# mohsij/spacecraft-pose-estimation

Hardware: AMD Instinct MI355X
Metric: poses/sec end-to-end (HRNet+PnP) at batch 256; keypoint/pose err vs ref (higher is better)
Workload: dtype bf16

## Files before the change

### spacecraft-pose-estimation_amd/csrc/api.cpp

```cpp
#include "common.h"
#include <new>

using namespace scpose;

struct scpose_conv { PackedConv pc; };

extern "C" int32_t scpose_abi_version(void) { return SCPOSE_ABI_VERSION; }
extern "C" int32_t scpose_is_dev_build(void) { return scpose::kDevBuild ? 1 : 0; }
extern "C" const char* scpose_last_error(void) { return last_error(); }

extern "C" int32_t scpose_decode(const float* heatmaps, int32_t n, int32_t j, int32_t h, int32_t w,
                                 const float* center, const float* scale, int32_t post_process,
                                 float* preds_xyc, void* stream) {
  if (n == 0) return SCPOSE_OK;
  SCP_REQUIRE(heatmaps && preds_xyc, "decode: null argument");
  return decode_launch(heatmaps, n, j, h, w, center, scale, post_process, preds_xyc, nullptr,
                       nullptr, static_cast<hipStream_t>(stream));
}

extern "C" int32_t scpose_crop_warp(const uint8_t* frames, const int64_t* offsets, const int32_t* frame_hw,
                                    const double* minv, int32_t n, int32_t out_h, int32_t out_w, int32_t swap_rb,
                                    uint8_t* crops, void* stream) {
  if (n == 0) return SCPOSE_OK;
  SCP_REQUIRE(frames && offsets && frame_hw && minv && crops, "crop_warp: null argument");
// ... 398 lines not shown
}

extern "C" int32_t scpose_conv_create(const float* weight, const float* bias, int32_t cout,
                                      int32_t cin, int32_t ksize, int32_t stride, int32_t dtype,
                                      scpose_conv_t* out) {
  SCP_REQUIRE(weight && out, "conv_create: null argument");
  scpose_conv* c = new (std::nothrow) scpose_conv();
  if (!c) { set_error("conv_create: out of host memory"); return SCPOSE_E_NOMEM; }
  const int32_t rc = conv_upload(weight, bias, cout, cin, ksize, stride, dtype, &c->pc);
  if (rc != SCPOSE_OK) { conv_free(&c->pc); delete c; return rc; }
  *out = c;
  return SCPOSE_OK;
}

extern "C" int32_t scpose_conv_destroy(scpose_conv_t c) {
  if (!c) return SCPOSE_OK;
  conv_free(&c->pc);
  delete c;
  return SCPOSE_OK;
}

extern "C" int32_t scpose_conv_forward(scpose_conv_t c, const void* in, int32_t n, int32_t h,
                                       int32_t w, const void* residual, int32_t relu,
                                       int32_t out_nchw_f32, void* out, void* stream) {
  SCP_REQUIRE(c && in && out, "conv_forward: null argument");
  return conv_launch(c->pc, in, n, h, w, residual, relu, out_nchw_f32, out,
                     static_cast<hipStream_t>(stream));
}

extern "C" int32_t scpose_basic_block_forward(scpose_conv_t conv1, scpose_conv_t conv2, const void* in, int32_t n,
                                              int32_t h, int32_t w, void* out, void* stream) {
  SCP_REQUIRE(conv1 && conv2 && in && out, "basic_block_forward: null argument");
  SCP_REQUIRE(block_fusable(conv1->pc, conv2->pc), "basic_block_forward: not a fusable pair (3x3 stride-1 C->C->C, C = 32 or 48)");
  return block_launch(conv1->pc, conv2->pc, in, n, h, w, out, static_cast<hipStream_t>(stream));
}

extern "C" int32_t scpose_fuse_sum(const void* const* terms, const int32_t* shifts, int32_t nterms,
                                   int32_t n, int32_t c, int32_t h, int32_t w, int32_t dtype,
                                   void* out, void* stream) {
  SCP_REQUIRE(terms && shifts && out, "fuse_sum: null argument");
  return fuse_sum_launch(terms, shifts, nterms, n, c, h, w, dtype, out,
                         static_cast<hipStream_t>(stream));
}

extern "C" int32_t scpose_nchw_f32_to_blocked(const float* src, int32_t n, int32_t c, int32_t h,
                                              int32_t w, int32_t dtype, void* dst, void* stream) {
  SCP_REQUIRE(src && dst, "nchw_f32_to_blocked: null argument");
  return nchw_to_blocked_launch(src, n, c, h, w, dtype, dst, static_cast<hipStream_t>(stream));
}

extern "C" int32_t scpose_blocked_to_nchw_f32(const void* src, int32_t n, int32_t c, int32_t h,
                                              int32_t w, int32_t dtype, float* dst, void* stream) {
  SCP_REQUIRE(src && dst, "blocked_to_nchw_f32: null argument");
  return blocked_to_nchw_launch(src, n, c, h, w, dtype, dst, static_cast<hipStream_t>(stream));
}
```

### spacecraft-pose-estimation_amd/csrc/common.h

```cpp
#pragma once
#include <hip/hip_runtime.h>
#include <stdint.h>
#include <stddef.h>
#include <string>
#include <vector>
#include <string.h>

#include "../../include/scpose.h"

namespace scpose {

void set_error(const char* fmt, ...);
const char* dev_env(const char* name);
const char* last_error();

#define SCP_CHECK_HIP(expr)                                                         \
  do {                                                                              \
    hipError_t _e = (expr);                                                         \
    if (_e != hipSuccess) {                                                         \
      ::scpose::set_error("%s failed: %s (%s:%d)", #expr, hipGetErrorString(_e),    \
                          __FILE__, __LINE__);                                      \
      return SCPOSE_E_HIP;                                                          \
    }                                                                               \
  } while (0)
// ... 109 lines not shown
  float* d_b1 = nullptr;
  size_t w1_bytes = 0;
  int cout_pad1 = 0;
  struct TileMemo { int n = -1, ho = 0, wo = 0, cus = 0; M32Tiling t; };
  mutable TileMemo m32_memo[2];
  void* d_ws2 = nullptr;
  float* d_bs2 = nullptr;
};
bool conv_s2r_config(int cin, int cout, int stride, int* planes, int* nblk, int* g);
size_t conv_s2r_pack(const float* w, int cout, int cin, int dtype, uint16_t* dst);
void conv_s2r_pack_bias(const float* bias, int cout, float* dst);
int32_t conv_s2r_launch(const PackedConv& pc, const void* in, int N, int H, int W, int relu, void* out, hipStream_t stream);
bool conv1x1_stream_eligible(const PackedConv& pc);
int32_t conv1x1_stream_launch(const PackedConv& pc, const void* in, int N, int H, int W, const void* res, int relu,
                              void* out, hipStream_t stream);

void choose_mrep_cp(int cin, int cout, int ks, int stride, int* mrep, int* cp);
void choose_tile(int ks, int stride, int Ho, int Wo, int* nrep, int* th, int* tw);

size_t pack_conv_weights(const float* w, int cout, int cin, int ks, int mt, int cp, int dtype,
                         uint16_t* dst, int* nchunks, int* ksteps_full);

int32_t conv_upload(const float* w, const float* bias, int cout, int cin, int ks, int stride,
                    int dtype, PackedConv* pc);
void conv_free(PackedConv* pc);
int32_t conv_launch(const PackedConv& pc, const void* in, int N, int H, int W, const void* res,
                    int relu, int out_nchw_f32, void* out, hipStream_t stream, int cu_share = 0);
size_t conv_lds_bytes(const PackedConv& pc, int nrep, int th, int tw);
int plane_stride_for(int stride, int halo_h, int halo_w);
int32_t conv_launch_pipe(const PackedConv& pc, ConvLaunch& L, int nrep, int nt, int occ, int groups, hipStream_t stream);
size_t conv_pipe_lds_bytes(const PackedConv& pc, int plane_stride, int groups);
const void* conv_zero_page();
bool block_fusable(const PackedConv& c1, const PackedConv& c2);
int32_t block_launch(const PackedConv& c1, const PackedConv& c2, const void* in, int N, int H, int W, void* out,
                     hipStream_t stream);
int conv_device_cus();
unsigned long long* conv_dbg_buffer(hipStream_t stream);
void conv_dbg_set_grid(int grid);
constexpr int kMrep48 = 15;
bool conv_m32_choose(int cin, int cout, int ks, int stride, int* mr, int* wm, int* cp);
size_t pack_conv_weights_m32(const float* w, int cout, int cin, int ks, int mt, int cp, int dtype,
                             uint16_t* dst, int* nchunks, int* ksteps_full);
int32_t conv_launch_m32(const PackedConv& pc, ConvLaunch& L, hipStream_t stream);

void stem_fused_pack(const float* w1, const float* b1, const float* w2, const float* b2, int dtype, std::vector<uint16_t>* pw1,
                     std::vector<uint16_t>* pw2, std::vector<float>* pb1, std::vector<float>* pb2);
int32_t stem_fused_launch(const void* in, int in_fmt, const void* w1, const void* w2, const float* b1, const float* b2,
                          const float* mean_std, int N, int H, int W, int dtype, void* out,
                          uint32_t* sched , hipStream_t stream);

bool bottleneck_fusable(int cin, int cmid, int cout);
void bottleneck_pack(const float* w1, const float* w2, const float* w3, const float* wds, const float* b1, const float* b2, const float* b3,
                     const float* bds, int cin, int dtype,
                     std::vector<uint16_t>* pw1, std::vector<uint16_t>* pw2, std::vector<uint16_t>* pw3, std::vector<float>* pb);
int32_t bottleneck_launch(const void* in, const void* w1, const void* w2, const void* w3, const float* bias, int N, int H, int W,
                          int cin, int dtype, void* out, uint32_t* sched ,
                          hipStream_t stream);

struct FuseDownPacked {
  void* d_w = nullptr;
  float* d_b = nullptr;
  int c0 = 0, nb = 0, dtype = 0;
};
bool fuse_down_supported(int nb, int c0, int c1);
int32_t fuse_down_upload(const float* w, const float* bias, int nb, int c0, int dtype, FuseDownPacked* fd);
void fuse_down_free(FuseDownPacked* fd);
int32_t fuse_down_launch(const FuseDownPacked& fd, const void* x0, int N, int H, int W, const void* const* terms, void* y,
                         void* const* outs, hipStream_t stream);
// ... 73 lines not shown
```

### spacecraft-pose-estimation_amd/csrc/conv_block.hip

```cpp
#include <stdlib.h>
#include <type_traits>

#include "conv_block2_kernel.h"

namespace scpose {

bool block_fusable(const PackedConv& c1, const PackedConv& c2) {
  static const char* e = dev_env("SCPOSE_FUSE_BLOCK");
  if (e && atoi(e) == 0) return false;
  const int C = c1.cin;
  return c1.variant == 0 && c2.variant == 0 && c1.ks == 3 && c2.ks == 3 && c1.stride == 1 && c2.stride == 1 &&
         c1.cout == C && c2.cin == C && c2.cout == C && (C == 48 || C == 32) && c1.mt == C && c2.mt == C &&
         c1.nchunks == 1 && c2.nchunks == 1 && c1.n_mblk == 1 && c2.n_mblk == 1 && c1.dtype == c2.dtype &&
         c1.ksteps_full == block_ksteps(C / 16) && block_lds_bytes(C / 16) <= 160 * 1024;
}

int32_t block_launch(const PackedConv& c1, const PackedConv& c2, const void* in, int N, int H, int W, void* out,
                     hipStream_t stream) {
  SCP_REQUIRE(block_fusable(c1, c2), "block: the two convolutions are not a fusable BasicBlock");
  SCP_REQUIRE(N > 0 && H > 0 && W > 0, "block: bad shape N=%d H=%d W=%d", N, H, W);
  BlockLaunch L;
  L.in = in; L.w1 = c1.d_w; L.w2 = c2.d_w; L.b1 = c1.d_bias; L.b2 = c2.d_bias; L.out = out;
  L.zero16 = conv_zero_page();
  SCP_REQUIRE(L.zero16, "block: cannot allocate the zero page");
  {
    static const char* e = dev_env("SCPOSE_M32_BUF");
    const size_t bytes = (size_t)N * (c1.cin / 8) * H * W * 16;
    L.bytes = (bytes < 0xfffffff0ull && !(e && atoi(e) == 0)) ? (uint32_t)bytes : 0;
  }
  L.N = N; L.H = H; L.W = W;
  L.tiles_x = (W + kBlockTile - 1) / kBlockTile;
  L.tiles_y = (H + kBlockTile - 1) / kBlockTile;
  L.tiles_total = N * L.tiles_x * L.tiles_y;
  L.fd_tiles_img = make_fastdiv(L.tiles_x * L.tiles_y);
  L.fd_tiles_x = make_fastdiv(L.tiles_x);
  int grid = conv_device_cus();
  if (grid > L.tiles_total) grid = L.tiles_total;
  L.tiles_per_wg = (L.tiles_total + grid - 1) / grid;
  L.grid = (L.tiles_total + L.tiles_per_wg - 1) / L.tiles_per_wg;
  { static const char* e = dev_env("SCPOSE_DBG"); const int dbg = (kDevBuild && e) ? atoi(e) : 0;
    L.dbg_buf = (dbg & 8) ? conv_dbg_buffer(stream) : nullptr;
    if (dbg & 8) conv_dbg_set_grid(L.grid); }
  const int mrep = c1.cin / 16;
  static const char* v1 = dev_env("SCPOSE_BLOCK_V1");
  if (L.bytes != 0 && !(v1 && atoi(v1))) {
    if (c1.dtype == SCPOSE_DT_BF16) return mrep == 3 ? block2_launch_one<0, 3>(L, stream) : block2_launch_one<0, 2>(L, stream);
    return mrep == 3 ? block2_launch_one<1, 3>(L, stream) : block2_launch_one<1, 2>(L, stream);
  }
  if (c1.dtype == SCPOSE_DT_BF16) {
    if (mrep == 3) return block_launch_one<0, 3>(L, stream);
    return block_launch_one<0, 2>(L, stream);
  }
  if (mrep == 3) return block_launch_one<1, 3>(L, stream);
  return block_launch_one<1, 2>(L, stream);
}

}
```

### spacecraft-pose-estimation_amd/csrc/conv_block2_kernel.h

```cpp
#pragma once
#include "conv_block_kernel.h"

namespace scpose {

constexpr size_t block2_lds_bytes(int mrep) { return 1024 + 2 * 2 * mrep * (size_t)(block_xs() + block_ms()) + (size_t)mrep * 256 * 16; }

template <int DT, int MREP>
__global__ __launch_bounds__(512, 2) void conv_block2_kernel(const BlockLaunch p) {
  extern __shared__ __attribute__((aligned(16))) char smem[];
  typedef typename DtOf<DT>::type T;
  typedef typename FragOf<T>::type frag_t;
  constexpr int MT = 16 * MREP, PLANES = 2 * MREP, KSTEPS = block_ksteps(MREP), NPT = MREP * 9;
  constexpr int XS = block_xs(), MS = block_ms();
  char* const xl0 = smem + 1024;
  char* const ml0 = xl0 + 2 * PLANES * XS;
  char* const rl0 = ml0 + 2 * PLANES * MS;

  const int tid = threadIdx.x, lane = tid & 63, wave = __builtin_amdgcn_readfirstlane(tid >> 6);
  const int q = lane >> 4, r = lane & 15, half = lane >> 5, psel = q & 1, hi = q >> 1;
  const int role = wave >> 2, rw = wave & 3, rtid = tid & 255;
  const int HW = p.H * p.W;
  const int tiles_per_img = p.tiles_x * p.tiles_y;

  const char* wsrc = static_cast<const char*>(role ? p.w2 : p.w1);
  frag_t wf[KSTEPS][MREP];
#pragma unroll
  for (int s = 0; s < KSTEPS; ++s)
#pragma unroll
    for (int m = 0; m < MREP; ++m)
      wf[s][m] = *reinterpret_cast<const frag_t*>(wsrc + (size_t)s * (4 * MT * 16) + (q * MT + m * 16 + r) * 16);
  float* const bias_l = reinterpret_cast<float*>(smem) + role * 64;
  if (tid < MT) { reinterpret_cast<float*>(smem)[tid] = p.b1[tid]; reinterpret_cast<float*>(smem)[64 + tid] = p.b2[tid]; }

  const int wg = xcd_remap(blockIdx.x, p.grid);
  const int t_begin = wg * p.tiles_per_wg;
  const int t_end = min(p.tiles_total, t_begin + p.tiles_per_wg);
  const int ntiles = t_end - t_begin;
  auto decode = [&](int t, int& img, int& oy0, int& ox0) {
    img = pipe_fdiv(t, p.fd_tiles_img);
    const int rem = t - img * tiles_per_img;
    const int ty = pipe_fdiv(rem, p.fd_tiles_x);
    oy0 = ty * kBlockTile; ox0 = (rem - ty * p.tiles_x) * kBlockTile;
  };
  const buf_rsrc_t rs_in = make_buf(p.in, p.bytes), rs_out = make_buf(p.out, p.bytes);

  auto x_voff = [&](int t, int i) -> uint32_t {
    int img, oy0, ox0;
    decode(t, img, oy0, ox0);
    int rt = rtid;
    asm volatile("" : "+v"(rt));
    const int slot = rt + 256 * i;
    const int hy = slot / 20, hx = slot - hy * 20;
    const int iy = oy0 - 2 + hy, ix = ox0 - 2 + hx;
    const bool ok = iy >= 0 && iy < p.H && ix >= 0 && ix < p.W;
    return ok ? (uint32_t)(img * PLANES * HW + iy * p.W + ix) * 16u : BUF_OOB;
  };
  auto x_dma = [&](uint32_t voff, int i, int pl, int b) {
    if (rtid + 256 * i < 400)
      dma16_buf(rs_in, voff, (uint32_t)(pl * HW) * 16u, xl0 + b * (PLANES * XS) + pl * XS + (rw * 64 + 256 * i) * 16);
  };
  auto issue_x = [&](int t, int b) {
#pragma unroll
    for (int i = 0; i < 2; ++i) {
      const uint32_t voff = x_voff(t, i);
#pragma unroll
      for (int pl = 0; pl < PLANES; ++pl) x_dma(voff, i, pl, b);
    }
  };

  auto koff = [](int pt, int PS, int ROWW) constexpr -> int {
    return pt < NPT ? 2 * (pt / 9) * PS + ((pt % 9) / 3 * ROWW + (pt % 9) % 3) * 16 : 0;
  };

  auto kloop = [&](auto ncol_c, auto role_c, const char* tile, const int* pixoff, f32x4 (*acc)[3], auto&& side, int psel_k) {
    constexpr int NCOL = decltype(ncol_c)::value;
    constexpr int ROLE = decltype(role_c)::value;
    constexpr int PS = ROLE ? MS : XS, ROWW = ROLE ? 18 : 20;
// ... 17 lines not shown
    static_for<0, KSTEPS>([&](auto sc) {
      constexpr int S = decltype(sc)::value;
      fetch(std::integral_constant<int, S + 2>{});
      __builtin_amdgcn_sched_barrier(0);
#pragma unroll
      for (int m = 0; m < MREP; ++m)
#pragma unroll
        for (int n = 0; n < NCOL; ++n) acc[m][n] = mfma16<T>(wf[S][m], bf[S % 3][n], acc[m][n]);
      side(sc);
      __builtin_amdgcn_sched_barrier(0);
    });
  };

  if (role == 1 && ntiles > 0) issue_x(t_begin, 0);
  asm volatile("s_waitcnt vmcnt(0)" ::: "memory");
  __syncthreads();

  unsigned long long tph[6] = {0, 0, 0, 0, 0, 0};
  auto now = [&]() -> unsigned long long {
    if (!SCP_DBG_BUF(p)) return 0ull;
    unsigned long long t;
    asm volatile("s_memtime %0\n\ts_waitcnt lgkmcnt(0)" : "=s"(t) : : "memory");
    return t;
  };
  if (role == 0) {
    for (int i = 0; i <= ntiles; ++i) {
      if (i < ntiles) {
        const int t = t_begin + i;
        int img, oy0, ox0;
        decode(t, img, oy0, ox0);
        const char* xl = xl0 + (i & 1) * (PLANES * XS);
        char* ml = ml0 + (i & 1) * (PLANES * MS);
        const bool narrow = i > 0 && ox0 > 0;
#pragma unroll 1
        for (int pass = 0; pass < 3; ++pass) {
          int rr = r;
          asm volatile("" : "+v"(rr));
          auto geom = [&](int n, int& pidx, int& my, int& mx) {
            const int c = rw + 4 * (2 * pass + n);
            pidx = narrow ? (c < 18 ? c * 18 + 2 + rr : 18 * 18) : c * 16 + rr;
            const bool ok = pidx < 18 * 18;
            my = ok ? pidx / 18 : 0;
            mx = ok ? pidx - my * 18 : 0;
          };
          const int cmax = narrow ? 18 : 21;
          const int ncol = (rw + 8 * pass < cmax) + (rw + 8 * pass + 4 < cmax);
          if (ncol == 0) continue;
          int pixoff[2];
#pragma unroll
          for (int n = 0; n < 2; ++n) {
            int pidx, my, mx;
            geom(n, pidx, my, mx);
            pixoff[n] = (my * 20 + mx) * 16;
          }
          f32x4 acc[MREP][3];
#pragma unroll
          for (int m = 0; m < MREP; ++m) {
            const float4 b4 = *reinterpret_cast<const float4*>(bias_l + m * 16 + q * 4);
#pragma unroll
            for (int n = 0; n < 2; ++n) acc[m][n] = f32x4{b4.x, b4.y, b4.z, b4.w};
          }
          const unsigned long long s1 = now();
          auto none = [](auto) {};
          if (ncol == 2) kloop(std::integral_constant<int, 2>{}, std::integral_constant<int, 0>{}, xl, pixoff, acc, none, psel);
          else kloop(std::integral_constant<int, 1>{}, std::integral_constant<int, 0>{}, xl, pixoff, acc, none, psel);
          const unsigned long long s2 = now();
          tph[1] += s2 - s1;
#pragma unroll
          for (int n = 0; n < 2; ++n) {
            int pidx, my, mx;
            asm volatile("" : "+v"(rr));
            geom(n, pidx, my, mx);
            const int gy = oy0 - 1 + my, gx = ox0 - 1 + mx;
            const bool inimg = gy >= 0 && gy < p.H && gx >= 0 && gx < p.W;
            const bool okn = pidx < 18 * 18 && n < ncol;
#pragma unroll
            for (int m = 0; m < MREP; ++m) {
              uint2 o;
              o.x = relu2_16(pack2<T>(acc[m][n][0], acc[m][n][1]), 0u);
              o.y = relu2_16(pack2<T>(acc[m][n][2], acc[m][n][3]), 0u);
              if (!inimg) o = make_uint2(0u, 0u);
              if (okn) *reinterpret_cast<uint2*>(ml + (2 * m + psel) * MS + pidx * 16 + 8 * hi) = o;
            }
          }
          tph[2] += now() - s2;
        }
      }
      const unsigned long long s9 = now();
      asm volatile("s_waitcnt lgkmcnt(0)\n\ts_barrier" ::: "memory");
      tph[5] += now() - s9;
    }
  } else {
    u32x4 res0[MREP];
#pragma unroll
    for (int m = 0; m < MREP; ++m) res0[m] = u32x4{0u, 0u, 0u, 0u};
    for (int i = 0; i <= ntiles; ++i) {
      const unsigned long long s0 = now();
      if (i == 0 && 1 < ntiles) issue_x(t_begin + 1, 1);
      if (i >= 1 && i < ntiles) {
        int img1, oy1, ox1;
        decode(t_begin + i, img1, oy1, ox1);
        int rt = rtid;
        asm volatile("" : "+v"(rt));
        if (ox1 > 0 && rt < PLANES * 36) {
          const int kpl = rt / 36, krem = rt - kpl * 36;
          const u32x4 keep = *reinterpret_cast<const u32x4*>(ml0 + ((i - 1) & 1) * (PLANES * MS) + kpl * MS + ((krem >> 1) * 18 + 16 + (krem & 1)) * 16);
          *reinterpret_cast<u32x4*>(ml0 + (i & 1) * (PLANES * MS) + kpl * MS + ((krem >> 1) * 18 + (krem & 1)) * 16) = keep;
        }
      }
      tph[0] += now() - s0;
      if (i >= 1) {
        const int t = t_begin + i - 1;
        int img, oy0, ox0;
        decode(t, img, oy0, ox0);
        const char* ml = ml0 + ((i - 1) & 1) * (PLANES * MS);
        auto conv2_pass = [&](auto pass_c) {
          constexpr int pass = decltype(pass_c)::value;
          const int row0 = rw + 8 * pass, row1 = row0 + 4;
          int rt2 = tid;
          asm volatile("" : "+v"(rt2));
          const int rr = rt2 & 15, half_ = (rt2 >> 5) & 1, psel_ = (rt2 >> 4) & 1;
          const int oy = oy0 + (half_ ? row1 : row0), ox = ox0 + rr;
// ... 95 lines not shown
```

### spacecraft-pose-estimation_amd/csrc/conv_block_kernel.h

```cpp
#pragma once
#include "common.h"
#include "conv_device.h"
#include "conv_pipe_kernel.h"

namespace scpose {

struct BlockLaunch {
  const void* in;
  const void* w1;
  const void* w2;
  const float* b1;
  const float* b2;
  void* out;
  const void* zero16;
  uint32_t bytes;
  int32_t N, H, W;
  int32_t tiles_x, tiles_y, tiles_total, tiles_per_wg, grid;
  FastDiv fd_tiles_img, fd_tiles_x;
  unsigned long long* dbg_buf;
};

template <int S, int E, typename F>
__device__ __forceinline__ void static_for(F&& f) {
  if constexpr (S < E) {
    f(std::integral_constant<int, S>{});
    static_for<S + 1, E>(f);
  }
}

constexpr int kBlockTile = 16;
constexpr int block_ksteps(int mrep) { return (mrep * 9 + 1) / 2; }
constexpr int block_xs() { return 20 * 20 * 16; }
constexpr int block_ms() { return (18 * 18 * 16 + 255) & ~255; }
constexpr size_t block_lds_bytes(int mrep) {
  return 1024 + 2 * (size_t)block_ksteps(mrep) * 4 * (16 * mrep) * 16 + 2 * mrep * (size_t)(block_xs() + block_ms());
}

template <int DT, int MREP>
__global__ __launch_bounds__(512, 2) void conv_block_kernel(const BlockLaunch p) {
  extern __shared__ __attribute__((aligned(16))) char smem[];
  typedef typename DtOf<DT>::type T;
  typedef typename FragOf<T>::type frag_t;
  constexpr int MT = 16 * MREP, PLANES = 2 * MREP, KSTEPS = block_ksteps(MREP), NPT = MREP * 9;
  constexpr int XS = block_xs(), MS = block_ms();
  constexpr int WBYTES = KSTEPS * 4 * MT * 16;

  int* koffA = reinterpret_cast<int*>(smem);
  int* koffB = koffA + 64;
  float* bias1 = reinterpret_cast<float*>(smem + 512);
  float* bias2 = bias1 + 64;
  char* w1l = smem + 1024;
  char* w2l = w1l + WBYTES;
// ... 275 lines not shown
```

### spacecraft-pose-estimation_amd/csrc/conv_pipe.hip

```cpp
#include <stdio.h>
#include <stdlib.h>
#include <vector>

#include "common.h"

namespace scpose {

int32_t conv_pipe_dispatch_bf16(int ks, int stride, int mrep, int nrep, int nt, int occ, const ConvLaunch& L, size_t lds, hipStream_t st);
int32_t conv_pipe_dispatch_f16(int ks, int stride, int mrep, int nrep, int nt, int occ, const ConvLaunch& L, size_t lds, hipStream_t st);

int32_t conv_stag_dispatch_bf16(int mrep, int nrep, const ConvLaunch& L, size_t lds, hipStream_t st);
int32_t conv_stag_dispatch_f16(int mrep, int nrep, const ConvLaunch& L, size_t lds, hipStream_t st);

static void* g_zero_page[16] = {nullptr};
static unsigned long long* g_dbg_buf = nullptr;
static int g_dbg_grid = 0;

const void* conv_zero_page() {
  int dev = 0;
  if (hipGetDevice(&dev) != hipSuccess || dev < 0 || dev >= 16) return nullptr;
  if (!g_zero_page[dev]) {
    void* p = nullptr;
    if (hipMalloc(&p, 256) != hipSuccess) return nullptr;
    if (hipMemset(p, 0, 256) != hipSuccess) return nullptr;
// ... 59 lines not shown
  L.items_per_wg = (L.items_total + grid - 1) / grid;
  L.grid = (L.items_total + L.items_per_wg - 1) / L.items_per_wg;
  g_dbg_grid = L.grid;
  if (groups == 2) {
    if (pc.dtype == SCPOSE_DT_BF16) return conv_stag_dispatch_bf16(pc.mrep, nrep, L, lds, stream);
    return conv_stag_dispatch_f16(pc.mrep, nrep, L, lds, stream);
  }
  if (pc.dtype == SCPOSE_DT_BF16) return conv_pipe_dispatch_bf16(pc.ks, pc.stride, pc.mrep, nrep, nt, occ, L, lds, stream);
  return conv_pipe_dispatch_f16(pc.ks, pc.stride, pc.mrep, nrep, nt, occ, L, lds, stream);
}

}

extern "C" void scpose_dbg_dump(void) {
  using namespace scpose;
  if (!g_dbg_buf || g_dbg_grid <= 0) return;
  (void)hipDeviceSynchronize();
  const int n = g_dbg_grid * 8 * 6;
  std::vector<unsigned long long> h(n);
  (void)hipMemcpy(h.data(), g_dbg_buf, n * 8, hipMemcpyDeviceToHost);
  const char* names[6] = {"setup+residual+DMA issue", "MFMA loop", "vmcnt wait", "finalize", "barrier", "stores"};
  double tot = 0, sum[6] = {0};
  int nw = 0;
  for (int i = 0; i < g_dbg_grid * 8; ++i) { double t = 0; for (int k = 0; k < 6; ++k) { sum[k] += (double)h[i * 6 + k]; t += (double)h[i * 6 + k]; } nw += t > 0; }
  for (int k = 0; k < 6; ++k) tot += sum[k];
  printf("  (%d workgroups, %d waves with stamps)\n", g_dbg_grid, nw);
  for (int k = 0; k < 6; ++k) printf("  %-26s %10.0f cycles/wave  %5.1f%%\n", names[k], sum[k] / (nw ? nw : 1), 100 * sum[k] / tot);
  for (int role = 0; role < 2; ++role) {
    double rs[6] = {0}; int rn = 0;
    for (int b = 0; b < g_dbg_grid; ++b)
      for (int w = role * 4; w < role * 4 + 4; ++w) { double t = 0; for (int k = 0; k < 6; ++k) { rs[k] += (double)h[(b * 8 + w) * 6 + k]; t += (double)h[(b * 8 + w) * 6 + k]; } rn += t > 0; }
    if (rn) { printf("  waves %d-%d:", role * 4, role * 4 + 3); for (int k = 0; k < 6; ++k) printf(" %9.0f", rs[k] / rn); printf("\n"); }
  }
}
```

### spacecraft-pose-estimation_amd/csrc/conv_pipe_kernel.h

```cpp
#pragma once
#include "common.h"
#include "conv_device.h"

namespace scpose {

typedef __attribute__((address_space(3))) void lds_void_t;
typedef const __attribute__((address_space(1))) void gbl_void_t;
typedef unsigned int u32x4 __attribute__((ext_vector_type(4)));

__device__ __forceinline__ int pipe_fdiv(int n, const FastDiv& f) {
  return (int)((__umulhi((uint32_t)n, f.mul) + (uint32_t)n * f.add) >> f.shift);
}

__device__ __forceinline__ void dma16(const void* g, void* l_wave_base) {
  __builtin_amdgcn_global_load_lds((gbl_void_t*)g, (lds_void_t*)l_wave_base, 16, 0, 0);
}

constexpr uint32_t BUF_OOB = 0xfffffff0u;
#if defined(__HIP_DEVICE_COMPILE__)
typedef __amdgpu_buffer_rsrc_t buf_rsrc_t;
__device__ __forceinline__ buf_rsrc_t make_buf(const void* base, uint32_t bytes) {
  return __builtin_amdgcn_make_buffer_rsrc(const_cast<void*>(base), 0, bytes, 0x00020000);
}
__device__ __forceinline__ void dma16_buf(buf_rsrc_t r, uint32_t voff, uint32_t soff, void* l_wave_base) {
  __builtin_amdgcn_raw_ptr_buffer_load_lds(r, (lds_void_t*)l_wave_base, 16, voff, soff, 0, 0);
}
__device__ __forceinline__ void store16_buf(buf_rsrc_t r, uint32_t voff, uint32_t soff, u32x4 v) {
  __builtin_amdgcn_raw_buffer_store_b128(v, r, voff, soff, 0);
  asm volatile("s_nop 1" ::"v"(v) : "memory");
}
__device__ __forceinline__ u32x4 load16_buf(buf_rsrc_t r, uint32_t voff, uint32_t soff) {
  return __builtin_amdgcn_raw_buffer_load_b128(r, voff, soff, 0);
}
__device__ __forceinline__ void store4_buf(buf_rsrc_t r, uint32_t voff, uint32_t v) {
  __builtin_amdgcn_raw_buffer_store_b32(v, r, voff, 0u, 0);
}
#else
struct buf_rsrc_t {};
__device__ inline buf_rsrc_t make_buf(const void*, uint32_t) { return buf_rsrc_t{}; }
__device__ inline void dma16_buf(buf_rsrc_t, uint32_t, uint32_t, void*) {}
__device__ inline void store16_buf(buf_rsrc_t, uint32_t, uint32_t, u32x4) {}
__device__ inline u32x4 load16_buf(buf_rsrc_t, uint32_t, uint32_t) { return u32x4{0u, 0u, 0u, 0u}; }
__device__ inline void store4_buf(buf_rsrc_t, uint32_t, uint32_t) {}
#endif

template <int DT, int KS, int STRIDE, int MREP, int NREP, int NT, int OCC, int G>
__global__ __launch_bounds__(256 * G, (G == 2) ? 2 : OCC) void conv_pipe_kernel(const ConvLaunch p) {
  static_assert(G == 1 || NT == 1, "parallel tile groups and sequential tile groups are exclusive");
  extern __shared__ __attribute__((aligned(16))) char smem[];
  typedef typename DtOf<DT>::type T;
  typedef typename FragOf<T>::type frag_t;
  constexpr int MT = 16 * MREP;
  constexpr int MAXP = (STRIDE == 1) ? 2 : 3;
  constexpr int KK = KS * KS;
  constexpr int NPAIR = (NREP + 1) / 2;

  int* koff = reinterpret_cast<int*>(smem);
  float* bias_l = reinterpret_cast<float*>(smem + 512);
  char* wl0 = smem + 512 + p.lds_bias;
  char* xl0 = wl0 + p.nbuf_w * p.lds_w;

  const int lane = threadIdx.x & 63;
  const int wave_all = __builtin_amdgcn_readfirstlane(threadIdx.x >> 6);
  const int grp = wave_all >> 2;
  const int wave = wave_all & 3, tid = threadIdx.x & 255;
  const int q = lane >> 4, r = lane & 15;
  const int HW = p.H * p.W;
  const int HP = p.halo_h * p.halo_w;
  const int npix = p.th * p.tw;
  const int planes_last = p.cin_planes - (p.nchunks - 1) * p.cp;
  const bool w_resident = p.nbuf_w == 1;

  if (threadIdx.x < 128) {
    const int tbl = threadIdx.x >> 6, e = threadIdx.x & 63;
// ... 442 lines not shown
```

### spacecraft-pose-estimation_amd/csrc/hrnet.cpp

```cpp
#include <math.h>
#include <stdio.h>
#include <stdarg.h>
#include <new>

#include <algorithm>
#include <map>
#include <string>
#include <vector>

#include "common.h"

namespace scpose {

static const double kBnEps = 1e-5;

struct HostTensor { const float* p; int64_t n; };

struct Weights {
  std::map<std::string, HostTensor> m;
  bool allow_missing;
  std::string missing;

  const float* get(const std::string& k, int64_t numel) {
    auto it = m.find(k);
// ... 51 lines not shown
  int epoch, lane;
  int par_kind;
};

}

struct scpose_hrnet_lanes {
  hipStream_t side[3] = {nullptr, nullptr, nullptr};
  std::vector<hipEvent_t> fork;
  std::vector<hipEvent_t> join;
  unsigned kinds = 0xe;
};

struct scpose_hrnet {
  scpose_hrnet_desc desc;
  int device = 0;
  std::vector<scpose::PackedConv> convs;
  float* d_mean_std = nullptr;
  void* d_stemf_w1 = nullptr;
  void* d_stemf_w2 = nullptr;
  float* d_stemf_b1 = nullptr;
  float* d_stemf_b2 = nullptr;
  struct Bneck { void* w1 = nullptr; void* w2 = nullptr; void* w3 = nullptr; float* bias = nullptr; int cin = 256; };
  std::vector<Bneck> bnecks;
  std::vector<scpose::FuseDownPacked> fdowns;
  float* d_head_bias = nullptr;
  uint32_t* d_sched = nullptr;
  int head_k = 0, head_s = 1;
  struct HeadFused { bool ok = false; int fuse_op = -1, conv_op = -1; void* d_w = nullptr; float* d_b = nullptr;
                     bool active = false; } headf;
  std::vector<scpose::TensorDesc> tensors;
  std::vector<scpose::Op> ops;
  std::vector<std::pair<std::string, int>> taps;
  struct Plan { int n = -1, h = -1, w = -1; size_t bytes = 0, part_off = 0; std::vector<size_t> off; } plan[2];
  std::vector<hipEvent_t> events;
  bool events_valid = false;
};

namespace scpose {

struct Builder {
  scpose_hrnet* net;
  Weights* W;
  int32_t status = SCPOSE_OK;
  int epoch = 0, lane = 0;
  bool serial = true;
  int par_kind = 0;
  void push(Op op) {
    if (serial) ++epoch;
    op.epoch = epoch; op.lane = serial ? 0 : lane; op.par_kind = serial ? 0 : par_kind;
    net->ops.push_back(op);
  }
  void parallel_begin(int kind) { ++epoch; serial = false; lane = 0; par_kind = kind; }
  void parallel_end() { serial = true; lane = 0; }

  int new_tensor(int C, int ds, const std::string& name) {
    net->tensors.push_back(TensorDesc{C, ds, -1});
    const int t = (int)net->tensors.size() - 1;
    if (!name.empty()) net->taps.emplace_back(name, t);
    return t;
  }
  void rename_tap(int t, const std::string& name) { for (auto& tp : net->taps) if (tp.second == t) tp.first = name; }
  void drop_tap(int t) {
    for (size_t i = 0; i < net->taps.size(); ++i) if (net->taps[i].second == t) { net->taps.erase(net->taps.begin() + i); --i; }
  }
  static std::string tensor_name(const std::string& cname) {
    return cname.size() > 2 && cname.compare(cname.size() - 2, 2, ".0") == 0 ? cname.substr(0, cname.size() - 2) : cname;
// ... 409 lines not shown
        for (size_t j = 0; j < freel.size() && !merged; ++j)
          if (i != j && freel[i].off + freel[i].size == freel[j].off) {
            freel[i].size += freel[j].size;
            freel.erase(freel.begin() + j);
            merged = true;
          }
    }
  };
  P.off.assign(net->tensors.size(), 0);
  std::vector<char> released(net->tensors.size(), 0);
  std::vector<int> pending;
  int cur_epoch = net->ops.empty() ? 0 : net->ops[0].epoch;
  for (size_t i = 0; i < net->ops.size(); ++i) {
    const Op& op = net->ops[i];
    if (mode == 1 && op.epoch != cur_epoch) {
      for (int t : pending) release(P.off[t], tensor_bytes(net->tensors[t], n, h, w));
      pending.clear();
      cur_epoch = op.epoch;
    }
    if (op.out >= 0) P.off[op.out] = alloc(tensor_bytes(net->tensors[op.out], n, h, w));
    for (int k = 0; k < op.nouts; ++k) P.off[op.outs[k]] = alloc(tensor_bytes(net->tensors[op.outs[k]], n, h, w));
    auto done = [&](int t) {
      if (t >= 0 && net->tensors[t].last_use == (int)i && !released[t]) {
        released[t] = 1;
        if (mode == 1) pending.push_back(t);
        else release(P.off[t], tensor_bytes(net->tensors[t], n, h, w));
      }
    };
    done(op.in); done(op.res);
    for (int k = 0; k < op.nterms; ++k) done(op.term[k]);
  }
  P.part_off = top;
  if (net->headf.ok) top += 2 * head_fused_part_bytes(n);
  P.n = n; P.h = h; P.w = w; P.bytes = top;
  return top;
}

struct HeadDecode {
  const float* center;
  const float* scale;
  int post_process;
  float* preds;
};

bool hrnet_tail_fused(const scpose_hrnet* net, int n, int h, int w) {
  if (!net->headf.ok) return false;
  static const char* e = dev_env("SCPOSE_NO_HEAD_FUSE");
  const Op& fo = net->ops[net->headf.fuse_op];
  const TensorDesc& ty = net->tensors[fo.out];
  return !(e && atoi(e)) && head_fused_supported(fo.nterms, ty.C, net->desc.num_joints, n, h >> ty.ds, w >> ty.ds);
}

int32_t hrnet_forward(scpose_hrnet* net, const void* in, int in_fmt, int n, int h, int w,
                      float* heatmaps, void* ws, size_t ws_bytes, hipStream_t st, bool profile, int stop_tensor = -1,
                      int mode = 0, const scpose_hrnet_lanes* lanes = nullptr, const HeadDecode* dec = nullptr) {
  SCP_REQUIRE(n > 0, "hrnet_forward: batch %d", n);
  const bool fused_tail = hrnet_tail_fused(net, n, h, w) && stop_tensor != net->ops[net->headf.fuse_op].out;
  net->headf.active = fused_tail;
  SCP_REQUIRE(heatmaps || (dec && fused_tail) || stop_tensor >= 0,
              "hrnet_forward: this network's tail is not fused for this shape -- key points need a heat-map buffer");
  SCP_REQUIRE(h % 32 == 0 && w % 32 == 0 && h > 0 && w > 0, "hrnet_forward: H=%d W=%d must be multiples of 32", h, w);
  const size_t need = hrnet_plan(net, n, h, w, mode);
  if (ws_bytes < need || !ws) {
    set_error("hrnet_forward: workspace %zu bytes < required %zu", ws_bytes, need);
    return SCPOSE_E_WORKSPACE;
  }
// ... 47 lines not shown
      const void* terms[4];
      for (int k = 0; k < fo.nterms; ++k) terms[k] = ptr(fo.term[k]);
      rc = head_fused_launch(terms, fo.shift, fo.nterms, n, ty.C, h >> ty.ds, w >> ty.ds, net->desc.num_joints, net->desc.dtype,
                             net->headf.d_w, net->headf.d_b, heatmaps, dec ? part_v : nullptr,
                             dec ? part_i : nullptr, dec ? dec->center : nullptr, dec ? dec->scale : nullptr,
                             dec ? dec->post_process : 0, dec ? dec->preds : nullptr, st);
    } else if (op.kind == OP_STEM2) {
      rc = stem_fused_launch(in, in_fmt, net->d_stemf_w1, net->d_stemf_w2, net->d_stemf_b1, net->d_stemf_b2, net->d_mean_std,
                             n, h, w, net->desc.dtype, ptr(op.out), net->d_sched + 16 * oi, st);
    } else if (op.kind == OP_CONV) {
      const TensorDesc& ti = net->tensors[op.in];
      void* out = op.out == -2 ? static_cast<void*>(heatmaps) : ptr(op.out);
      rc = conv_launch(net->convs[op.conv], ptr(op.in), n, h >> ti.ds, w >> ti.ds, ptr(op.res),
                       op.relu, op.out_f32, out, st, open_lanes ? conv_device_cus() / 2 : 0);
    } else if (op.kind == OP_HEAD) {
      const TensorDesc& ti = net->tensors[op.in];
      float* out = op.out == -2 ? heatmaps : static_cast<float*>(ptr(op.out));
      rc = head_gather_launch(ptr(op.in), net->d_head_bias + op.head * 16, static_cast<const float*>(ptr(op.res)), n,
                              net->desc.num_joints, h >> ti.ds, w >> ti.ds, net->head_k, net->head_s,
                              net->desc.dtype, out, st);
    } else if (op.kind == OP_BNECK) {
      const TensorDesc& ti = net->tensors[op.in];
      const scpose_hrnet::Bneck& bn = net->bnecks[op.conv];
      rc = bottleneck_launch(ptr(op.in), bn.w1, bn.w2, bn.w3, bn.bias, n, h >> ti.ds, w >> ti.ds, bn.cin, net->desc.dtype, ptr(op.out), net->d_sched + 16 * oi, st);
    } else if (op.kind == OP_FDOWN) {
      const TensorDesc& ti = net->tensors[op.in];
      const void* terms[3] = {nullptr, nullptr, nullptr};
      void* outs[3] = {nullptr, nullptr, nullptr};
      for (int k = 0; k < op.nterms; ++k) terms[k] = ptr(op.term[k]);
      for (int k = 0; k < op.nouts; ++k) outs[k] = ptr(op.outs[k]);
      rc = fuse_down_launch(net->fdowns[op.conv], ptr(op.in), n, h >> ti.ds, w >> ti.ds, terms, ptr(op.out), outs, st);
    } else if (op.kind == OP_BLOCK) {
      const TensorDesc& ti = net->tensors[op.in];
      rc = block_launch(net->convs[op.conv], net->convs[op.conv2], ptr(op.in), n, h >> ti.ds, w >> ti.ds, ptr(op.out), st);
    } else {
      const TensorDesc& to = net->tensors[op.out];
      const void* terms[4];
      for (int k = 0; k < op.nterms; ++k) terms[k] = ptr(op.term[k]);
      rc = fuse_sum_launch(terms, op.shift, op.nterms, n, to.C, h >> to.ds, w >> to.ds,
                           net->desc.dtype, ptr(op.out), st);
    }
    if (rc != SCPOSE_OK) return rc;
    if (stop_tensor >= 0 && (op.out == stop_tensor || (op.nouts > 0 && std::find(op.outs, op.outs + op.nouts, stop_tensor) != op.outs + op.nouts)))
      break;
  }
  if (lanes) { const int32_t rc = join_lanes(); if (rc != SCPOSE_OK) return rc; }
  st = st0;
  if (dec && !fused_tail && stop_tensor < 0) {
    int32_t hh = 0, hw = 0;
    hh = h / 4 * net->head_s; hw = w / 4 * net->head_s;
    const int32_t rc = decode_launch(heatmaps, n, net->desc.num_joints, hh, hw, dec->center, dec->scale, dec->post_process,
                                     dec->preds, nullptr, nullptr, st);
    if (rc != SCPOSE_OK) return rc;
  }
  if (profile) {
    SCP_CHECK_HIP(hipEventRecord(net->events[opi], st));
    net->events_valid = true;
  }
  return SCPOSE_OK;
}

static void op_work(const scpose_hrnet* net, const Op& op, int h, int w, double* f, double* by, int32_t sig[4], bool unfused = false) {
  *f = 0; *by = 0;
  sig[0] = op.kind; sig[1] = sig[2] = sig[3] = 0;
  if (!unfused && net->headf.active && &op == &net->ops[net->headf.fuse_op]) {
    const TensorDesc& to = net->tensors[op.out];
    sig[1] = op.nterms; sig[2] = to.C; sig[3] = to.C;
// ... 381 lines not shown
```

Measured before the change: 9830.

## Carry halo rows of fused BasicBlock intermediate between vertically adjacent tiles

In the fused two-conv BasicBlock kernel, each workgroup now saves the bottom two rows of its conv1 intermediate tile to a per-workgroup global strip buffer. When it later processes the tile directly below, it DMAs those rows back into LDS instead of recomputing them, so fewer halo columns/passes of conv1 are computed. This adds strip stores, a vmcnt wait at the barrier, scratch buffer planning per lane, and a stream-keyed allocator for the standalone API. It also adds a per-wave debug print.

Result: no change. 9892 (median of 6 runs) (+0.6%).

```diff
diff --git a/spacecraft-pose-estimation_amd/csrc/api.cpp b/spacecraft-pose-estimation_amd/csrc/api.cpp
--- a/spacecraft-pose-estimation_amd/csrc/api.cpp
+++ b/spacecraft-pose-estimation_amd/csrc/api.cpp
@@ -454,7 +454,10 @@
                                               int32_t h, int32_t w, void* out, void* stream) {
   SCP_REQUIRE(conv1 && conv2 && in && out, "basic_block_forward: null argument");
   SCP_REQUIRE(block_fusable(conv1->pc, conv2->pc), "basic_block_forward: not a fusable pair (3x3 stride-1 C->C->C, C = 32 or 48)");
-  return block_launch(conv1->pc, conv2->pc, in, n, h, w, out, static_cast<hipStream_t>(stream));
+  const size_t strip_bytes = block_strip_bytes(conv1->pc.cin, n, h, w);
+  void* strip = strip_bytes ? block_strip_scratch(static_cast<hipStream_t>(stream), strip_bytes) : nullptr;
+  SCP_REQUIRE(!strip_bytes || strip, "basic_block_forward: cannot allocate %zu bytes of scratch", strip_bytes);
+  return block_launch(conv1->pc, conv2->pc, in, n, h, w, out, strip, strip_bytes, static_cast<hipStream_t>(stream));
 }
 
 extern "C" int32_t scpose_fuse_sum(const void* const* terms, const int32_t* shifts, int32_t nterms,
diff --git a/spacecraft-pose-estimation_amd/csrc/common.h b/spacecraft-pose-estimation_amd/csrc/common.h
--- a/spacecraft-pose-estimation_amd/csrc/common.h
+++ b/spacecraft-pose-estimation_amd/csrc/common.h
@@ -165,8 +165,10 @@
 size_t conv_pipe_lds_bytes(const PackedConv& pc, int plane_stride, int groups);
 const void* conv_zero_page();
 bool block_fusable(const PackedConv& c1, const PackedConv& c2);
+size_t block_strip_bytes(int C, int N, int H, int W);
+void* block_strip_scratch(hipStream_t stream, size_t bytes);
 int32_t block_launch(const PackedConv& c1, const PackedConv& c2, const void* in, int N, int H, int W, void* out,
-                     hipStream_t stream);
+                     void* strip, size_t strip_bytes, hipStream_t stream);
 int conv_device_cus();
 unsigned long long* conv_dbg_buffer(hipStream_t stream);
 void conv_dbg_set_grid(int grid);
diff --git a/spacecraft-pose-estimation_amd/csrc/conv_block.hip b/spacecraft-pose-estimation_amd/csrc/conv_block.hip
--- a/spacecraft-pose-estimation_amd/csrc/conv_block.hip
+++ b/spacecraft-pose-estimation_amd/csrc/conv_block.hip
@@ -1,4 +1,6 @@
 #include <stdlib.h>
+#include <map>
+#include <mutex>
 #include <type_traits>
 
 #include "conv_block2_kernel.h"
@@ -15,8 +17,43 @@
          c1.ksteps_full == block_ksteps(C / 16) && block_lds_bytes(C / 16) <= 160 * 1024;
 }
 
+static void block_grid(int N, int H, int W, BlockLaunch& L) {
+  L.tiles_x = (W + kBlockTile - 1) / kBlockTile;
+  L.tiles_y = (H + kBlockTile - 1) / kBlockTile;
+  L.tiles_total = N * L.tiles_x * L.tiles_y;
+  int grid = conv_device_cus();
+  if (grid > L.tiles_total) grid = L.tiles_total;
+  L.tiles_per_wg = (L.tiles_total + grid - 1) / grid;
+  L.grid = (L.tiles_total + L.tiles_per_wg - 1) / L.tiles_per_wg;
+}
+
+size_t block_strip_bytes(int C, int N, int H, int W) {
+  if (N <= 0 || H <= 0 || W <= 0) return 0;
+  BlockLaunch L;
+  block_grid(N, H, W, L);
+  if (L.tiles_y < 2 || L.tiles_per_wg <= L.tiles_x) return 0;
+  return (size_t)L.grid * 2 * (C / 8) * 2 * (L.tiles_x * kBlockTile + 2) * 16;
+}
+
+void* block_strip_scratch(hipStream_t stream, size_t bytes) {
+  struct Buf { void* p = nullptr; size_t cap = 0; };
+  static std::mutex mu;
+  static std::map<std::pair<int, hipStream_t>, Buf> bufs;
+  int dev = 0;
+  if (hipGetDevice(&dev) != hipSuccess) return nullptr;
+  std::lock_guard<std::mutex> lock(mu);
+  Buf& b = bufs[std::make_pair(dev, stream)];
+  if (b.cap < bytes) {
+    if (b.p) (void)hipFree(b.p);
+    b.p = nullptr; b.cap = 0;
+    if (hipMalloc(&b.p, bytes) != hipSuccess) { b.p = nullptr; return nullptr; }
+    b.cap = bytes;
+  }
+  return b.p;
+}
+
 int32_t block_launch(const PackedConv& c1, const PackedConv& c2, const void* in, int N, int H, int W, void* out,
-                     hipStream_t stream) {
+                     void* strip, size_t strip_bytes, hipStream_t stream) {
   SCP_REQUIRE(block_fusable(c1, c2), "block: the two convolutions are not a fusable BasicBlock");
   SCP_REQUIRE(N > 0 && H > 0 && W > 0, "block: bad shape N=%d H=%d W=%d", N, H, W);
   BlockLaunch L;
@@ -29,15 +66,17 @@
     L.bytes = (bytes < 0xfffffff0ull && !(e && atoi(e) == 0)) ? (uint32_t)bytes : 0;
   }
   L.N = N; L.H = H; L.W = W;
-  L.tiles_x = (W + kBlockTile - 1) / kBlockTile;
-  L.tiles_y = (H + kBlockTile - 1) / kBlockTile;
-  L.tiles_total = N * L.tiles_x * L.tiles_y;
+  block_grid(N, H, W, L);
   L.fd_tiles_img = make_fastdiv(L.tiles_x * L.tiles_y);
   L.fd_tiles_x = make_fastdiv(L.tiles_x);
-  int grid = conv_device_cus();
-  if (grid > L.tiles_total) grid = L.tiles_total;
-  L.tiles_per_wg = (L.tiles_total + grid - 1) / grid;
-  L.grid = (L.tiles_total + L.tiles_per_wg - 1) / L.tiles_per_wg;
+  {
+    static const char* e = dev_env("SCPOSE_BLOCK_CARRY");
+    const size_t need = block_strip_bytes(c1.cin, N, H, W);
+    SCP_REQUIRE(need == 0 || (strip && strip_bytes >= need), "block: strip of %zu bytes, %zu needed", strip_bytes, need);
+    const bool on = need != 0 && !(e && atoi(e) == 0);
+    L.strip = on ? strip : nullptr;
+    L.strip_bytes = on ? (uint32_t)need : 0u;
+  }
   { static const char* e = dev_env("SCPOSE_DBG"); const int dbg = (kDevBuild && e) ? atoi(e) : 0;
     L.dbg_buf = (dbg & 8) ? conv_dbg_buffer(stream) : nullptr;
     if (dbg & 8) conv_dbg_set_grid(L.grid); }
diff --git a/spacecraft-pose-estimation_amd/csrc/conv_block2_kernel.h b/spacecraft-pose-estimation_amd/csrc/conv_block2_kernel.h
--- a/spacecraft-pose-estimation_amd/csrc/conv_block2_kernel.h
+++ b/spacecraft-pose-estimation_amd/csrc/conv_block2_kernel.h
@@ -43,6 +43,11 @@
     oy0 = ty * kBlockTile; ox0 = (rem - ty * p.tiles_x) * kBlockTile;
   };
   const buf_rsrc_t rs_in = make_buf(p.in, p.bytes), rs_out = make_buf(p.out, p.bytes);
+  const int SW = p.tiles_x * kBlockTile + 2;
+  const uint32_t strip_plane = (uint32_t)(2 * SW) * 16u, strip_half = PLANES * strip_plane;
+  const uint32_t strip_wg = blockIdx.x * 2u * strip_half;
+  const buf_rsrc_t rs_strip = make_buf(p.strip, p.strip_bytes);
+  const bool carry_on = p.strip != nullptr;
 
   auto x_voff = [&](int t, int i) -> uint32_t {
     int img, oy0, ox0;
@@ -126,18 +131,34 @@
         const char* xl = xl0 + (i & 1) * (PLANES * XS);
         char* ml = ml0 + (i & 1) * (PLANES * MS);
         const bool narrow = i > 0 && ox0 > 0;
+        const bool carry = carry_on && oy0 > 0 && i >= p.tiles_x;
+        const bool keep = carry_on && oy0 + kBlockTile < p.H && i + p.tiles_x < ntiles;
+        if (carry) {
+          int ll = lane;
+          asm volatile("" : "+v"(ll));
+          const int row = ll >= 18 ? 1 : 0, col = ll - 18 * row;
+          const uint32_t voff = (uint32_t)(row * SW + ox0 + col) * 16u;
+          const uint32_t sbase = strip_wg + ((((oy0 >> 4) - 1) & 1) ? strip_half : 0u);
+          if (ll < 36) {
+            dma16_buf_l2(rs_strip, voff, sbase + rw * strip_plane, ml + rw * MS);
+            if (rw + 4 < PLANES) dma16_buf_l2(rs_strip, voff, sbase + (rw + 4) * strip_plane, ml + (rw + 4) * MS);
+          }
+        }
+        const int cmax = narrow ? (carry ? 16 : 18) : (carry ? 18 : 21);
+        const int npass = (cmax + 7) >> 3;
+        const int row_first = carry ? 2 : 0;
+        const uint32_t keep_base = strip_wg + (((oy0 >> 4) & 1) ? strip_half : 0u);
 #pragma unroll 1
-        for (int pass = 0; pass < 3; ++pass) {
+        for (int pass = 0; pass < npass; ++pass) {
           int rr = r;
           asm volatile("" : "+v"(rr));
           auto geom = [&](int n, int& pidx, int& my, int& mx) {
             const int c = rw + 4 * (2 * pass + n);
-            pidx = narrow ? (c < 18 ? c * 18 + 2 + rr : 18 * 18) : c * 16 + rr;
+            pidx = c >= cmax ? 18 * 18 : narrow ? (c + row_first) * 18 + 2 + rr : row_first * 18 + c * 16 + rr;
             const bool ok = pidx < 18 * 18;
             my = ok ? pidx / 18 : 0;
             mx = ok ? pidx - my * 18 : 0;
           };
-          const int cmax = narrow ? 18 : 21;
           const int ncol = (rw + 8 * pass < cmax) + (rw + 8 * pass + 4 < cmax);
           if (ncol == 0) continue;
           int pixoff[2];
@@ -168,6 +189,8 @@
             const int gy = oy0 - 1 + my, gx = ox0 - 1 + mx;
             const bool inimg = gy >= 0 && gy < p.H && gx >= 0 && gx < p.W;
             const bool okn = pidx < 18 * 18 && n < ncol;
+            const bool kept = keep && okn && my >= 16;
+            const uint32_t svoff = kept ? (uint32_t)((my - 16) * SW + gx + 1) * 16u + (uint32_t)(8 * hi) + (psel ? strip_plane : 0u) : BUF_OOB;
 #pragma unroll
             for (int m = 0; m < MREP; ++m) {
               uint2 o;
@@ -175,13 +198,14 @@
               o.y = relu2_16(pack2<T>(acc[m][n][2], acc[m][n][3]), 0u);
               if (!inimg) o = make_uint2(0u, 0u);
               if (okn) *reinterpret_cast<uint2*>(ml + (2 * m + psel) * MS + pidx * 16 + 8 * hi) = o;
+              if (kept) store8_buf(rs_strip, svoff, keep_base + (uint32_t)(2 * m) * strip_plane, o);
             }
           }
           tph[2] += now() - s2;
         }
       }
       const unsigned long long s9 = now();
-      asm volatile("s_waitcnt lgkmcnt(0)\n\ts_barrier" ::: "memory");
+      asm volatile("s_waitcnt vmcnt(0) lgkmcnt(0)\n\ts_barrier" ::: "memory");
       tph[5] += now() - s9;
     }
   } else {
diff --git a/spacecraft-pose-estimation_amd/csrc/conv_block_kernel.h b/spacecraft-pose-estimation_amd/csrc/conv_block_kernel.h
--- a/spacecraft-pose-estimation_amd/csrc/conv_block_kernel.h
+++ b/spacecraft-pose-estimation_amd/csrc/conv_block_kernel.h
@@ -18,6 +18,8 @@
   int32_t tiles_x, tiles_y, tiles_total, tiles_per_wg, grid;
   FastDiv fd_tiles_img, fd_tiles_x;
   unsigned long long* dbg_buf;
+  void* strip;
+  uint32_t strip_bytes;
 };
 
 template <int S, int E, typename F>
diff --git a/spacecraft-pose-estimation_amd/csrc/conv_pipe.hip b/spacecraft-pose-estimation_amd/csrc/conv_pipe.hip
--- a/spacecraft-pose-estimation_amd/csrc/conv_pipe.hip
+++ b/spacecraft-pose-estimation_amd/csrc/conv_pipe.hip
@@ -115,4 +115,9 @@
       for (int w = role * 4; w < role * 4 + 4; ++w) { double t = 0; for (int k = 0; k < 6; ++k) { rs[k] += (double)h[(b * 8 + w) * 6 + k]; t += (double)h[(b * 8 + w) * 6 + k]; } rn += t > 0; }
     if (rn) { printf("  waves %d-%d:", role * 4, role * 4 + 3); for (int k = 0; k < 6; ++k) printf(" %9.0f", rs[k] / rn); printf("\n"); }
   }
+  for (int w = 0; w < 8; ++w) {
+    double ws[6] = {0}; int wn = 0;
+    for (int b = 0; b < g_dbg_grid; ++b) { double t = 0; for (int k = 0; k < 6; ++k) { ws[k] += (double)h[(b * 8 + w) * 6 + k]; t += (double)h[(b * 8 + w) * 6 + k]; } wn += t > 0; }
+    if (wn) { printf("  wave %d:   ", w); for (int k = 0; k < 6; ++k) printf(" %9.0f", ws[k] / wn); printf("\n"); }
+  }
 }
diff --git a/spacecraft-pose-estimation_amd/csrc/conv_pipe_kernel.h b/spacecraft-pose-estimation_amd/csrc/conv_pipe_kernel.h
--- a/spacecraft-pose-estimation_amd/csrc/conv_pipe_kernel.h
+++ b/spacecraft-pose-estimation_amd/csrc/conv_pipe_kernel.h
@@ -25,9 +25,18 @@
 __device__ __forceinline__ void dma16_buf(buf_rsrc_t r, uint32_t voff, uint32_t soff, void* l_wave_base) {
   __builtin_amdgcn_raw_ptr_buffer_load_lds(r, (lds_void_t*)l_wave_base, 16, voff, soff, 0, 0);
 }
+__device__ __forceinline__ void dma16_buf_l2(buf_rsrc_t r, uint32_t voff, uint32_t soff, void* l_wave_base) {
+  __builtin_amdgcn_raw_ptr_buffer_load_lds(r, (lds_void_t*)l_wave_base, 16, voff, soff, 0, 16);
+}
 __device__ __forceinline__ void store16_buf(buf_rsrc_t r, uint32_t voff, uint32_t soff, u32x4 v) {
   __builtin_amdgcn_raw_buffer_store_b128(v, r, voff, soff, 0);
   asm volatile("s_nop 1" ::"v"(v) : "memory");
+}
+typedef uint32_t u32x2_t __attribute__((ext_vector_type(2)));
+__device__ __forceinline__ void store8_buf(buf_rsrc_t r, uint32_t voff, uint32_t soff, uint2 v) {
+  const u32x2_t d = {v.x, v.y};
+  __builtin_amdgcn_raw_buffer_store_b64(d, r, voff, soff, 0);
+  asm volatile("s_nop 1" ::"v"(d) : "memory");
 }
 __device__ __forceinline__ u32x4 load16_buf(buf_rsrc_t r, uint32_t voff, uint32_t soff) {
   return __builtin_amdgcn_raw_buffer_load_b128(r, voff, soff, 0);
@@ -39,7 +48,9 @@
 struct buf_rsrc_t {};
 __device__ inline buf_rsrc_t make_buf(const void*, uint32_t) { return buf_rsrc_t{}; }
 __device__ inline void dma16_buf(buf_rsrc_t, uint32_t, uint32_t, void*) {}
+__device__ inline void dma16_buf_l2(buf_rsrc_t, uint32_t, uint32_t, void*) {}
 __device__ inline void store16_buf(buf_rsrc_t, uint32_t, uint32_t, u32x4) {}
+__device__ inline void store8_buf(buf_rsrc_t, uint32_t, uint32_t, uint2) {}
 __device__ inline u32x4 load16_buf(buf_rsrc_t, uint32_t, uint32_t) { return u32x4{0u, 0u, 0u, 0u}; }
 __device__ inline void store4_buf(buf_rsrc_t, uint32_t, uint32_t) {}
 #endif
diff --git a/spacecraft-pose-estimation_amd/csrc/hrnet.cpp b/spacecraft-pose-estimation_amd/csrc/hrnet.cpp
--- a/spacecraft-pose-estimation_amd/csrc/hrnet.cpp
+++ b/spacecraft-pose-estimation_amd/csrc/hrnet.cpp
@@ -107,7 +107,7 @@
   std::vector<scpose::TensorDesc> tensors;
   std::vector<scpose::Op> ops;
   std::vector<std::pair<std::string, int>> taps;
-  struct Plan { int n = -1, h = -1, w = -1; size_t bytes = 0, part_off = 0; std::vector<size_t> off; } plan[2];
+  struct Plan { int n = -1, h = -1, w = -1; size_t bytes = 0, part_off = 0, strip_off[4] = {0, 0, 0, 0}, strip_bytes[4] = {0, 0, 0, 0}; std::vector<size_t> off; } plan[2];
   std::vector<hipEvent_t> events;
   bool events_valid = false;
 };
@@ -583,6 +583,14 @@
   }
   P.part_off = top;
   if (net->headf.ok) top += 2 * head_fused_part_bytes(n);
+  for (int l = 0; l < 4; ++l) P.strip_bytes[l] = 0;
+  for (const Op& op : net->ops)
+    if (op.kind == OP_BLOCK) {
+      const TensorDesc& ti = net->tensors[op.in];
+      const int l = op.lane >= 0 && op.lane < 4 ? op.lane : 0;
+      P.strip_bytes[l] = std::max(P.strip_bytes[l], block_strip_bytes(net->convs[op.conv].cin, n, h >> ti.ds, w >> ti.ds));
+    }
+  for (int l = 0; l < 4; ++l) { P.strip_off[l] = top; top += (P.strip_bytes[l] + 255) & ~(size_t)255; }
   P.n = n; P.h = h; P.w = w; P.bytes = top;
   return top;
 }
@@ -696,7 +704,9 @@
       rc = fuse_down_launch(net->fdowns[op.conv], ptr(op.in), n, h >> ti.ds, w >> ti.ds, terms, ptr(op.out), outs, st);
     } else if (op.kind == OP_BLOCK) {
       const TensorDesc& ti = net->tensors[op.in];
-      rc = block_launch(net->convs[op.conv], net->convs[op.conv2], ptr(op.in), n, h >> ti.ds, w >> ti.ds, ptr(op.out), st);
+      const int sl = op.lane >= 0 && op.lane < 4 ? op.lane : 0;
+      rc = block_launch(net->convs[op.conv], net->convs[op.conv2], ptr(op.in), n, h >> ti.ds, w >> ti.ds, ptr(op.out),
+                        base + net->plan[mode].strip_off[sl], net->plan[mode].strip_bytes[sl], st);
     } else {
       const TensorDesc& to = net->tensors[op.out];
       const void* terms[4];
```
